# yuxiaoxiangyong/Multilateral-Temporal-view-Pyramid-Transformer-for-Video-Inpainting-Detection

Measured on AMD Instinct MI355X. Metric: clips/sec fwd (B=8,T=5,224x224), higher is better.
Workload: dtype f32; 1 GPU; full Mumpy forward (3 temporal views, pyramid decoder), B=8 clips/GPU, T=5, 224x224, fp32, tubelets (5,4,1); global_batch=8, launch=hipGraph replay, fork/join over HIP streams (independent branches co-scheduled), parallelism=batch-sharded x1, one metric all-reduce

## Files before the change

### multilateral-temporal-view-pyramid-transformer-for-video-inpainting-detection_amd/csrc/gemm.hip

```cpp
#include <stdlib.h>
#include "common.h"
#include "gemm_ws.h"
#include "gemm_ws64.h"
using namespace mumpy;

namespace {

constexpr int BK = 32;
constexpr int LDR = 36;

struct ConvGeom {
    int H, W, Cin, kh, kw, ph, pw;
    int kseg, kstride;
};

__device__ __attribute__((aligned(128))) float g_zero_page[32];

template <int TM, int TN, int WM, int WN, bool OUT16 = false>
__device__ __forceinline__ void store_tile(const f32x16 (&acc)[TM][TN], int64_t m0, int n0, int wm, int wn, int c, int h,
                                           int64_t M, int N, const float* __restrict__ bias, const float* residual,
                                           float* Y, int act, int ksplit, int ks, float* slab) {
    const int wm_u = __builtin_amdgcn_readfirstlane(wm), wn_u = __builtin_amdgcn_readfirstlane(wn);
    const int64_t mw = m0 + wm_u * WM;
    const int64_t wbase = mw * N + n0 + wn_u * WN;
// ... 429 lines not shown
                        acc[i][j] = __builtin_amdgcn_mfma_f32_32x32x16_bf16(af[i][st][NP > 1 ? PA[q] : 0],
                                                                            bf[j][st][NP > 1 ? PB[q] : 0], acc[i][j], 0, 0, 0);
    };
    const int klast = kbeg + (nk - 1) * BK;
    if (NBUF == 2) {
        gload(kbeg);
        lstore(0);
        __syncthreads();
        for (int kc = 0; kc + 1 < nk; ++kc) {
            gload(kbeg + (kc + 1) * BK);
            __builtin_amdgcn_sched_barrier(0);
            fread(kc & 1);
            mma();
            lstore((kc & 1) ^ 1);
            __syncthreads();
        }
        fread((nk - 1) & 1);
        mma();
    } else {
        gload(kbeg);
        lstore(0);
        gload(nk > 1 ? kbeg + BK : kbeg);
        __syncthreads();
        for (int kc = 0; kc + 1 < nk; ++kc) {
            fread(0);
            __syncthreads();
            lstore(0);
            const int knext = kbeg + (kc + 2) * BK;
            gload(knext < klast ? knext : klast);
            mma();
            __syncthreads();
        }
        fread(0);
        mma();
    }
    store_tile<TM, TN, WM, WN, OUT16>(acc, m0, n0, wm, wn, c, h, M, N, bias, residual, Y, act, ksplit, ks, slab);
}

__global__ __launch_bounds__(256) void splitk_reduce_kernel(const float* __restrict__ slab, const float* __restrict__ bias,
                                                            const float* residual, float* Y, int64_t MN4, int N,
                                                            int ksplit, int act) {
    for (int64_t i = (int64_t)blockIdx.x * 256 + threadIdx.x; i < MN4; i += (int64_t)gridDim.x * 256) {
        f32x4 v = ordered_sum(reinterpret_cast<const f32x4*>(slab)[i], reinterpret_cast<const f32x4*>(slab) + MN4 + i, MN4, ksplit - 1);
        const int n = (int)((i * 4) % N);
        if (bias) v += *reinterpret_cast<const f32x4*>(bias + n);
        if (act == MUMPY_ACT_GELU) {
#pragma unroll
            for (int e = 0; e < 4; ++e) v[e] = gelu_erf(v[e]);
        }
        if (residual) v += reinterpret_cast<const f32x4*>(residual)[i];
        reinterpret_cast<f32x4*>(Y)[i] = v;
    }
}

struct Plan {
    int tile;
    int ksplit;
    unsigned gn;
    int64_t gm;
};

constexpr int NUM_CU = 256;

Plan make_plan_x3(int64_t M, int N, int K, bool allow_split) {
    Plan p;
    const int64_t gm128 = (M + 127) / 128, gm64 = (M + 63) / 64;
    const unsigned gn128 = (N + 127) / 128, gn64 = (N + 63) / 64;
    const int64_t b128 = gm128 * gn128, b64 = gm64 * gn64;
    auto fit = [&](int ks) {
        if (!allow_split) return 1;
        if (ks > K / 384) ks = K / 384;
        if (ks > 16) ks = 16;
        while (ks > 1 && (K % (32 * ks)) != 0) --ks;
        return ks < 1 ? 1 : ks;
    };
    const int ksw = fit((int)((448 + b128 / 2) / b128));
    if (b128 * ksw >= 240) {
        p.tile = 0; p.ksplit = ksw; p.gm = gm128; p.gn = gn128;
    } else {
        p.tile = 2; p.ksplit = (b64 < 2 * 256 && K >= 768) ? fit((int)((3 * 256 + b64 - 1) / b64)) : 1;
        p.gm = gm64; p.gn = gn64;
    }
    return p;
}

Plan make_plan(int64_t M, int N, int K, bool allow_split, bool x3 = false) {
    static const char* force = tune_str("MUMPY_GEMM_FORCE");
    if (x3 && !force) return make_plan_x3(M, N, K, allow_split);
    Plan p;
    const int64_t gm128 = (M + 127) / 128, gm64 = (M + 63) / 64;
    const unsigned gn128 = (N + 127) / 128, gn64 = (N + 63) / 64;
    const int64_t b128 = gm128 * gn128, b64 = gm64 * gn64;
    const double nk = (double)K / BK;
    const double t128 = (double)((b128 + NUM_CU - 1) / NUM_CU) * (nk + 2.0) / nk;
    double t64 = (double)((b64 + NUM_CU - 1) / NUM_CU) * 0.272;
    if (t64 < 0.357) t64 = 0.357;
    t64 *= (nk + 0.5) / nk;
    int tile = (t128 <= t64) ? 0 : 2;
    if (tile == 0 && b128 > NUM_CU && K >= 512) tile = 3;
    int ks = 1;
    static const int min_slice = tune_int("MUMPY_GEMM_MINSLICE", 384), max_ks = tune_int("MUMPY_GEMM_MAXKS", 16),
                     min_k = tune_int("MUMPY_GEMM_SPLIT_MINK", 768);
    if (tile == 2 && allow_split && b64 < 2 * NUM_CU && K >= min_k) {
        ks = (int)((3 * NUM_CU + b64 - 1) / b64);
        if (ks > K / min_slice) ks = K / min_slice;
        if (ks > max_ks) ks = max_ks;
        while (ks > 1 && (K % (32 * ks)) != 0) --ks;
        if (ks < 1) ks = 1;
    }
    if (force) {
        int ft = -1, fk = -1;
        if (sscanf(force, "%d,%d", &ft, &fk) >= 1 && ft >= 0 && ft <= 3) {
            tile = ft;
            if (fk >= 1 && allow_split && K % (32 * fk) == 0) ks = fk; else if (fk >= 1) ks = 1;
        }
    }
    p.tile = tile; p.ksplit = ks;
    p.gm = (tile == 0 || tile == 3) ? gm128 : gm64;
    p.gn = (tile == 2) ? gn64 : gn128;
    return p;
}

int device_cus() {
    static int num_cu = 0;
    if (!num_cu) {
        int dev = 0;
        hipDeviceProp_t prop;
        if (hipGetDevice(&dev) == hipSuccess && hipGetDeviceProperties(&prop, dev) == hipSuccess) num_cu = prop.multiProcessorCount;
        else num_cu = NUM_CU;
    }
    return num_cu;
}

int ws_plan(int64_t M, int N, int K, bool have_ws, bool conv) {
    static const int ws_mode = tune_int("MUMPY_GEMM_WS", 2);
    const int num_cu = device_cus();
    const int64_t tiles = ((M + 127) / 128) * ((N + 127) / 128);
    const int nk = K / 32;
    const double rounds = (double)tiles / num_cu, eff = rounds / (double)((tiles + num_cu - 1) / num_cu);
    const double per_cu = (double)tiles * nk / num_cu;
    int how = 0;
    if (ws_mode == 1) how = 1;
    else if (ws_mode == 3) how = have_ws ? 2 : 1;
    else if (ws_mode == 2 && conv) {
        if (have_ws && eff < 0.86 && per_cu >= 24.0 && (double)nk / per_cu <= 3.0) how = 2;
        else if (tiles >= (int64_t)(0.75 * num_cu) && eff >= 0.75 && K >= 128) how = 1;
    } else if (ws_mode == 2) {
        if (tiles >= (int64_t)(0.75 * num_cu) && eff >= 0.86 && K >= 128 && !(K >= 1024 && rounds >= 1.8)) how = 1;
        else if (have_ws && eff < 0.86 && per_cu >= 24.0 && (double)nk / per_cu <= 3.0 && !(K >= 1024 && rounds >= 1.8)) how = 2;
    }
    return how;
}

int launch_linear(const float* x, const float* W, const float* bias, const float* residual, float* y, int64_t M, int N,
                  int K, int act, float* ws, int64_t ws_bytes, hipStream_t s, int64_t rpb = 0, int64_t bstride = 0,
                  const ConvGeom* conv = nullptr, bool ws_clean = false, const gemm_ws::LnArgs* ln = nullptr, int kseg = 0,
                  int kstride = 0) {
    if (rpb <= 0) { rpb = M; bstride = 0; }
    ConvGeom cg = conv ? *conv : ConvGeom{0, 0, 0, 0, 0, 0, 0, 0, 0};
    cg.kseg = kseg; cg.kstride = kstride;
    const bool math_bf16 = (act & MUMPY_MATH_BF16) != 0;
    const bool math_x2 = (act & MUMPY_MATH_BF16X2) != 0;
    const bool math_x3 = (act & MUMPY_MATH_BF16X3) != 0 || math_x2;
    act &= 0xff;
    const gemm_ws::Conv cvd{cg.H, cg.W, cg.Cin, cg.kh, cg.kw};
    if (ln && (rpb < M || math_bf16 || math_x3 || conv || !gemm_ws::eligible(M, N, K) ||
               !ws_plan(M, N, K, ws && ws_bytes >= gemm_ws::workspace_bytes(device_cus()), false))) {
        set_error("linear: LayerNorm folding needs a shape the persistent 128x128 kernel takes (mumpy_linear_ln_tiles) in fp32 mode");
        return MUMPY_EINVAL;
    }
    if (rpb >= M && !kseg && !math_bf16 && !math_x3 && (conv ? gemm_ws::conv_eligible(M, N, cvd) : gemm_ws::eligible(M, N, K))) {
        const int num_cu = device_cus();
        const bool have_ws = ws && ws_bytes >= gemm_ws::workspace_bytes(num_cu);
        const int how = ws_plan(M, N, K, have_ws, conv != nullptr);
        const int nk = K / 32;
        static const int ws64_mode = tune_int("MUMPY_GEMM_WS64", 1);
        if (!how && !conv && ws64_mode) {
            const int64_t t64 = ((M + 63) / 64) * ((N + 63) / 64);
            const double r64 = (double)t64 / (2.0 * num_cu);
            const bool fits = ws64_mode == 2 || (act != MUMPY_ACT_GELU && nk <= 32 && t64 >= 64 && (r64 <= 1.0 || r64 >= 2.5 || nk <= 12));
            if (fits) {
                if (int rc = gemm_ws64::launch(x, W, bias, residual, y, M, N, K, act, num_cu, s)) return rc;
                MUMPY_CHECK_LAUNCH("linear(ws64)");
                return 0;
            }
        }
        if (how) {
            if (int rc = gemm_ws::launch(x, W, bias, residual, y, M, N, K, act, num_cu, s, ws, ws_bytes, how == 2 ? 1 : 0, nullptr, ws_clean,
                                         conv ? &cvd : nullptr, ln)) return rc;
            MUMPY_CHECK_LAUNCH("linear(ws)");
            return 0;
        }
    }
    Plan p = make_plan(M, N, K, ws != nullptr, math_x3);
    if (ws) { ws += 1024; ws_bytes -= 4096; }
    if (p.ksplit > 1 && (int64_t)p.ksplit * M * N * (int64_t)sizeof(float) > ws_bytes) p.ksplit = 1;
    const int64_t grid = p.gm * p.gn * p.ksplit;
    MUMPY_REQUIRE(grid < (1ll << 31), MUMPY_ERANGE, "linear: too many tiles");
#define MUMPY_GEMM(BM_, BN_, WM_, WN_, CV_)                                                                        \
    if (use_glds)                                                                                                  \
        hipLaunchKernelGGL((linear_kernel<BM_, BN_, WM_, WN_, CV_, true>), dim3((unsigned)grid),                     \
                           dim3(64 * (BM_ / WM_) * (BN_ / WN_)), 0, s, x, W, bias, residual, y, M, N, K, act, p.gn,  \
                           p.ksplit, ws, rpb, bstride, cg);                                               \
    else                                                                                                           \
    hipLaunchKernelGGL((linear_kernel<BM_, BN_, WM_, WN_, CV_, false>), dim3((unsigned)grid),                        \
                       dim3(64 * (BM_ / WM_) * (BN_ / WN_)), 0, s, x, W, bias, residual, y, M, N, K, act, p.gn, p.ksplit, \
                       ws, rpb, bstride, cg)
    static const bool use_glds = tune_int("MUMPY_GEMM_GLDS", 0) != 0;
    if (math_x3) {
        const bool wide = (p.tile == 0 || p.tile == 3);
#define MUMPY_GEMM_X3(BM_, BN_, WM_, WN_, CV_, NB_)                                                                    \
    hipLaunchKernelGGL((linear_bf16_kernel<BM_, BN_, WM_, WN_, CV_, 3, NB_>), dim3((unsigned)grid), dim3(256), 0, s, x, W, \
                       bias, residual, y, M, N, K, act, p.gn, p.ksplit, ws, rpb, bstride, cg)
#define MUMPY_GEMM_X2(BM_, BN_, WM_, WN_, CV_, NB_)                                                                    \
    hipLaunchKernelGGL((linear_bf16_kernel<BM_, BN_, WM_, WN_, CV_, 2, NB_>), dim3((unsigned)grid), dim3(256), 0, s, x, W, \
                       bias, residual, y, M, N, K, act, p.gn, p.ksplit, ws, rpb, bstride, cg)
        if (math_x2) {
            if (wide && conv) MUMPY_GEMM_X2(128, 128, 64, 64, true, 1);
            else if (wide) MUMPY_GEMM_X2(128, 128, 64, 64, false, 1);
            else if (conv) MUMPY_GEMM_X2(64, 64, 32, 32, true, 2);
            else MUMPY_GEMM_X2(64, 64, 32, 32, false, 2);
        }
        else if (wide && conv) MUMPY_GEMM_X3(128, 128, 64, 64, true, 1);
        else if (wide) MUMPY_GEMM_X3(128, 128, 64, 64, false, 1);
        else if (conv) MUMPY_GEMM_X3(64, 64, 32, 32, true, 2);
        else MUMPY_GEMM_X3(64, 64, 32, 32, false, 2);
#undef MUMPY_GEMM_X3
#undef MUMPY_GEMM_X2
    } else if (math_bf16) {
        const bool wide = (p.tile == 0 || p.tile == 3);
#define MUMPY_GEMM_H(BM_, BN_, WM_, WN_, CV_)                                                                          \
    hipLaunchKernelGGL((linear_bf16_kernel<BM_, BN_, WM_, WN_, CV_>), dim3((unsigned)grid), dim3(256), 0, s, x, W, bias,   \
                       residual, y, M, N, K, act, p.gn, p.ksplit, ws, rpb, bstride, cg)
        if (wide && conv) MUMPY_GEMM_H(128, 128, 64, 64, true);
        else if (wide) MUMPY_GEMM_H(128, 128, 64, 64, false);
        else if (conv) MUMPY_GEMM_H(64, 64, 32, 32, true);
        else MUMPY_GEMM_H(64, 64, 32, 32, false);
#undef MUMPY_GEMM_H
    } else if (p.tile == 3) {
        if (conv)
            hipLaunchKernelGGL((linear_kernel<128, 128, 64, 64, true, true, false>), dim3((unsigned)grid), dim3(256), 0, s, x, W,
                               bias, residual, y, M, N, K, act, p.gn, p.ksplit, ws, rpb, bstride, cg);
        else
            hipLaunchKernelGGL((linear_kernel<128, 128, 64, 64, false, true, false>), dim3((unsigned)grid), dim3(256), 0, s, x, W,
                               bias, residual, y, M, N, K, act, p.gn, p.ksplit, ws, rpb, bstride, cg);
    } else if (conv) {
        if (p.tile == 0) MUMPY_GEMM(128, 128, 64, 32, true);
        else if (p.tile == 1) MUMPY_GEMM(64, 128, 32, 64, true);
        else MUMPY_GEMM(64, 64, 32, 32, true);
    } else {
        if (p.tile == 0) MUMPY_GEMM(128, 128, 64, 32, false);
        else if (p.tile == 1) MUMPY_GEMM(64, 128, 32, 64, false);
        else MUMPY_GEMM(64, 64, 32, 32, false);
    }
#undef MUMPY_GEMM
    MUMPY_CHECK_LAUNCH("linear");
    if (p.ksplit > 1) {
        const int64_t mn4 = M * N / 4;
        int64_t g = (mn4 + 255) / 256;
        if (g > 2048) g = 2048;
        hipLaunchKernelGGL(splitk_reduce_kernel, dim3((unsigned)g), dim3(256), 0, s, ws, bias, residual, y, mn4, N,
                           p.ksplit, act);
        MUMPY_CHECK_LAUNCH("linear(split-K reduce)");
    }
    return 0;
}

}

static int check_linear_args(const float* x, const float* W, const float* residual, const float* y, int64_t M, int N,
                             int K, int act) {
    MUMPY_REQUIRE(x && W && y, MUMPY_ENULL, "linear: null pointer");
    MUMPY_REQUIRE(aligned16(x) && aligned16(W) && aligned16(y) && aligned16(residual), MUMPY_EALIGN,
                  "linear: pointers must be 16-byte aligned");
    MUMPY_REQUIRE(M < (1ll << 31) - 256 && (int64_t)N * 4 * 128 < (1ll << 32), MUMPY_ERANGE,
                  "linear: M=%lld rows / N=%d columns beyond the 32-bit row index / tile byte offsets", (long long)M, N);
    MUMPY_REQUIRE(M >= 0 && N > 0 && K > 0 && K % BK == 0 && N % 32 == 0, MUMPY_EINVAL,
                  "linear: need K %% 32 == 0 and N %% 32 == 0 (got M=%lld N=%d K=%d)", (long long)M, N, K);
    MUMPY_REQUIRE((act & 0xff) == MUMPY_ACT_NONE || (act & 0xff) == MUMPY_ACT_GELU, MUMPY_EINVAL, "linear: unknown act %d", act);
    constexpr int math_bits = MUMPY_MATH_BF16 | MUMPY_MATH_BF16X3 | MUMPY_MATH_BF16X2;
    MUMPY_REQUIRE((act & ~(0xff | math_bits)) == 0, MUMPY_EINVAL, "linear: unknown flag bits in act 0x%x", act);
    MUMPY_REQUIRE(((act & math_bits) & ((act & math_bits) - 1)) == 0, MUMPY_EINVAL, "linear: the MUMPY_MATH_* modes are exclusive");
    return 0;
}

extern "C" int mumpy_linear_fwd(const float* x, const float* W, const float* bias, const float* residual, float* y,
                                int64_t M, int N, int K, int act, void* stream) {
    if (M == 0) return 0;
    if (int rc = check_linear_args(x, W, residual, y, M, N, K, act)) return rc;
    return launch_linear(x, W, bias, residual, y, M, N, K, act, nullptr, 0, as_stream(stream));
}

extern "C" int64_t mumpy_linear_workspace_bytes(int64_t M, int N, int K) {
    if (M <= 0 || N <= 0 || K <= 0 || K % BK) return 0;
    const Plan p = make_plan(M, N, K, true), q = make_plan(M, N, K, true, true);
    const int ks = p.ksplit > q.ksplit ? p.ksplit : q.ksplit;
    int64_t bytes = ks > 1 ? (int64_t)ks * M * N * (int64_t)sizeof(float) + 4096 : 0;
    if (gemm_ws::eligible(M, N, K)) {
        const int64_t tiles = ((M + 127) / 128) * ((N + 127) / 128);
        const double per_cu = (double)tiles * (K / 32) / NUM_CU;
        const int64_t need = gemm_ws::workspace_bytes(2 * NUM_CU);
        if (per_cu >= 16.0 && bytes < need) bytes = need;
    }
    return bytes;
}

extern "C" int mumpy_linear_ws_fwd(const float* x, const float* W, const float* bias, const float* residual, float* y,
                                   int64_t M, int N, int K, int act, void* workspace, int64_t workspace_bytes,
                                   void* stream) {
    if (M == 0) return 0;
    if (int rc = check_linear_args(x, W, residual, y, M, N, K, act)) return rc;
    MUMPY_REQUIRE(aligned16(workspace), MUMPY_EALIGN, "linear: workspace must be 16-byte aligned");
    return launch_linear(x, W, bias, residual, y, M, N, K, act, static_cast<float*>(workspace),
                         workspace ? workspace_bytes : 0, as_stream(stream));
}

extern "C" int mumpy_linear_bf16s_fwd(const void* x, const void* W, const float* bias, const float* residual, void* y,
                                      int64_t M, int N, int K, int act, int out_bf16, void* stream) {
    if (M == 0) return 0;
    MUMPY_REQUIRE(x && W && y, MUMPY_ENULL, "linear_bf16s: null pointer");
    MUMPY_REQUIRE(aligned16(x) && aligned16(W) && aligned16(y) && aligned16(residual), MUMPY_EALIGN,
                  "linear_bf16s: pointers must be 16-byte aligned");
    MUMPY_REQUIRE(M > 0 && M < (1ll << 31) - 256 && (int64_t)N * 4 * 128 < (1ll << 32), MUMPY_ERANGE, "linear_bf16s: M=%lld / N=%d out of range", (long long)M, N);
    MUMPY_REQUIRE(N > 0 && K > 0 && K % BK == 0 && N % 32 == 0, MUMPY_EINVAL, "linear_bf16s: need K %% 32 == 0 and N %% 32 == 0 (got N=%d K=%d)", N, K);
    MUMPY_REQUIRE(act == MUMPY_ACT_NONE || act == MUMPY_ACT_GELU, MUMPY_EINVAL, "linear_bf16s: unknown act %d", act);
    const float* xf = static_cast<const float*>(x);
    const float* wf = static_cast<const float*>(W);
    float* yf = static_cast<float*>(y);
    const ConvGeom cg{0, 0, 0, 0, 0, 0, 0, 0, 0};
    hipStream_t s = as_stream(stream);
    MUMPY_REQUIRE(!(out_bf16 && residual), MUMPY_EINVAL, "linear_bf16s: a bf16 output takes no residual");
    {
        static const int ws16 = tune_int("MUMPY_GEMM_WS16", 2);
        static int num_cu = 0;
        if (!num_cu) {
            int dev = 0;
            hipDeviceProp_t prop;
            if (hipGetDevice(&dev) == hipSuccess && hipGetDeviceProperties(&prop, dev) == hipSuccess) num_cu = prop.multiProcessorCount;
            else num_cu = NUM_CU;
        }
        const int64_t tiles = ((M + 127) / 128) * ((N + 127) / 128);
        const double rounds = (double)tiles / num_cu, eff = rounds / (double)((tiles + num_cu - 1) / num_cu);
        if (ws16 && gemm_ws::eligible16(M, N, K) && (ws16 == 2 || (tiles >= (int64_t)(0.75 * num_cu) && eff >= 0.75))) {
            if (int rc = gemm_ws::launch16(x, W, bias, residual, y, M, N, K, act, out_bf16 != 0, num_cu, s)) return rc;
            MUMPY_CHECK_LAUNCH("linear_bf16s(ws)");
            return 0;
        }
    }
    const int64_t gm128 = (M + 127) / 128, gm64 = (M + 63) / 64;
    const unsigned gn128 = (N + 127) / 128, gn64 = (N + 63) / 64;
    const bool wide = gm128 * gn128 >= 200;
    const unsigned gn = wide ? gn128 : gn64;
    const int64_t grid = (wide ? gm128 : gm64) * gn;
    MUMPY_REQUIRE(grid < (1ll << 31), MUMPY_ERANGE, "linear_bf16s: too many tiles");
#define MUMPY_GEMM_S(BM_, BN_, WM_, WN_, O16_)                                                                             \
    hipLaunchKernelGGL((linear_bf16_kernel<BM_, BN_, WM_, WN_, false, 1, 2, true, O16_>), dim3((unsigned)grid), dim3(256), 0, s, \
                       xf, wf, bias, residual, yf, M, N, K, act, gn, 1, nullptr, M, (int64_t)0, cg)
    if (wide && out_bf16) MUMPY_GEMM_S(128, 128, 64, 64, true);
    else if (wide) MUMPY_GEMM_S(128, 128, 64, 64, false);
    else if (out_bf16) MUMPY_GEMM_S(64, 64, 32, 32, true);
    else MUMPY_GEMM_S(64, 64, 32, 32, false);
#undef MUMPY_GEMM_S
    MUMPY_CHECK_LAUNCH("linear_bf16s");
    return 0;
}

extern "C" int mumpy_linear_wsz_fwd(const float* x, const float* W, const float* bias, const float* residual, float* y,
                                    int64_t M, int N, int K, int act, void* workspace, int64_t workspace_bytes,
                                    void* stream) {
    if (M == 0) return 0;
    if (int rc = check_linear_args(x, W, residual, y, M, N, K, act)) return rc;
    MUMPY_REQUIRE(aligned16(workspace), MUMPY_EALIGN, "linear: workspace must be 16-byte aligned");
    return launch_linear(x, W, bias, residual, y, M, N, K, act, static_cast<float*>(workspace),
                         workspace ? workspace_bytes : 0, as_stream(stream), 0, 0, nullptr, true);
}

extern "C" int mumpy_workspace_status(const void* workspace, int* status) {
    MUMPY_REQUIRE(workspace && status, MUMPY_ENULL, "workspace_status: null pointer");
    unsigned w[2] = {0, 0};
    static_assert(gemm_ws::LN_GUARD_WORD + 1 == gemm_ws::STATUS_WORD, "status words must be adjacent");
    hipError_t e = hipMemcpy(w, static_cast<const unsigned*>(workspace) + gemm_ws::LN_GUARD_WORD, sizeof(w), hipMemcpyDeviceToHost);
    if (e != hipSuccess) { set_error("workspace_status: %s", hipGetErrorString(e)); return (int)e; }
    *status = w[1] ? (int)w[1] : (w[0] ? -1 : 0);
    return 0;
}

extern "C" int mumpy_linear_ln_tiles(int64_t M, int N, int K) {
    if (M <= 0 || N <= 0 || K <= 0 || K % BK || N % 32 || !gemm_ws::eligible(M, N, K)) return 0;
    return ws_plan(M, N, K, true, false) ? (N + 127) / 128 : 0;
}

extern "C" int mumpy_linear_lnx_fwd(const float* x, const float* W, const float* bias, const float* residual, float* y, int64_t M,
                                    int N, int K, int act, void* workspace, int64_t workspace_bytes, float* stats_out,
                                    const float* ln_stats, int ln_gn, const float* ln_colsum, float ln_eps, void* stream) {
    if (M == 0) return 0;
    if (int rc = check_linear_args(x, W, residual, y, M, N, K, act)) return rc;
    MUMPY_REQUIRE((act & ~0xff) == 0, MUMPY_EINVAL, "linear_lnx: fp32 matrix math only");
    MUMPY_REQUIRE(aligned16(workspace) && workspace, MUMPY_EALIGN, "linear_lnx: needs the kept (zeroed) workspace of mumpy_linear_wsz_fwd");
    MUMPY_REQUIRE((stats_out != nullptr) != (ln_stats != nullptr), MUMPY_EINVAL, "linear_lnx: exactly one of stats_out (producer) / ln_stats (consumer)");
    MUMPY_REQUIRE(!ln_stats || (ln_colsum && bias && !residual && ln_gn == (K + 127) / 128 && ln_gn <= 16 && ln_eps > 0.f), MUMPY_EINVAL,
                  "linear_lnx: the consumer takes W gamma, colsum, bias = W beta + b, no residual, and ln_gn = ceil(K / 128) tiles (got %d)", ln_gn);
    MUMPY_REQUIRE(aligned16(stats_out) && aligned16(ln_stats) && aligned16(ln_colsum), MUMPY_EALIGN, "linear_lnx: pointers must be 16-byte aligned");
    MUMPY_REQUIRE(M * (int64_t)((N + 127) / 128) * 8 < (1ll << 31) && M * (int64_t)(ln_gn > 0 ? ln_gn : 1) * 8 < (1ll << 31), MUMPY_ERANGE,
                  "linear_lnx: statistics buffer beyond 2 GiB");
    const gemm_ws::LnArgs ln{stats_out, ln_stats, ln_colsum, ln_gn, K, ln_eps};
    return launch_linear(x, W, bias, residual, y, M, N, K, act, static_cast<float*>(workspace), workspace_bytes, as_stream(stream), 0, 0,
                         nullptr, true, &ln);
}

extern "C" int mumpy_linear_rows_fwd(const float* x, int64_t rows_per_block, int64_t block_stride, const float* W,
                                     const float* bias, const float* residual, float* y, int64_t M, int N, int K, int act,
                                     void* workspace, int64_t workspace_bytes, void* stream) {
    if (M == 0) return 0;
    if (int rc = check_linear_args(x, W, residual, y, M, N, K, act)) return rc;
    MUMPY_REQUIRE(rows_per_block > 0 && M % rows_per_block == 0 && block_stride % 4 == 0, MUMPY_EINVAL,
                  "linear_rows: M=%lld must be a multiple of rows_per_block=%lld and block_stride %% 4 == 0",
                  (long long)M, (long long)rows_per_block);
    return launch_linear(x, W, bias, residual, y, M, N, K, act, static_cast<float*>(workspace),
                         workspace ? workspace_bytes : 0, as_stream(stream), rows_per_block, block_stride);
}

extern "C" int mumpy_linear_rows_kseg_fwd(const float* x, int64_t rows_per_block, int64_t block_stride, int kseg, int kstride,
                                          const float* W, const float* bias, const float* residual, float* y, int64_t M, int N, int K,
                                          int act, void* workspace, int64_t workspace_bytes, void* stream) {
    if (M == 0) return 0;
    if (int rc = check_linear_args(x, W, residual, y, M, N, K, act)) return rc;
    MUMPY_REQUIRE(rows_per_block > 0 && M % rows_per_block == 0 && block_stride % 4 == 0, MUMPY_EINVAL,
                  "linear_rows_kseg: M=%lld must be a multiple of rows_per_block=%lld and block_stride %% 4 == 0",
                  (long long)M, (long long)rows_per_block);
    MUMPY_REQUIRE(kseg > 0 && kseg % 32 == 0 && K % kseg == 0 && kstride % 4 == 0 && kstride >= 0, MUMPY_EINVAL,
                  "linear_rows_kseg: need kseg %% 32 == 0, K %% kseg == 0, kstride %% 4 == 0 (got kseg=%d K=%d kstride=%d)", kseg, K, kstride);
    return launch_linear(x, W, bias, residual, y, M, N, K, act, static_cast<float*>(workspace), workspace ? workspace_bytes : 0,
                         as_stream(stream), rows_per_block, block_stride, nullptr, false, nullptr, kseg, kstride);
}

extern "C" int64_t mumpy_conv2d_workspace_bytes(int B, int H, int W, int Cin, int Cout, int kh, int kw) {
    return mumpy_linear_workspace_bytes((int64_t)B * H * W, Cout, kh * kw * Cin);
}

extern "C" int mumpy_conv2d_nhwc_fwd(const float* x, const float* w_krsc, const float* bias, const float* residual,
                                     float* y, int B, int H, int W, int Cin, int Cout, int kh, int kw, int act,
                                     void* workspace, int64_t workspace_bytes, void* stream) {
    MUMPY_REQUIRE(B > 0 && H > 0 && W > 0 && H < 32768 && W < 32768, MUMPY_EINVAL, "conv2d: bad image size %dx%d", H, W);
    MUMPY_REQUIRE(kh > 0 && kw > 0 && (kh & 1) && (kw & 1), MUMPY_EINVAL, "conv2d: kernel %dx%d must be odd (same padding)", kh, kw);
    MUMPY_REQUIRE(Cin % 32 == 0 && Cout % 32 == 0, MUMPY_EINVAL, "conv2d: Cin=%d and Cout=%d must be multiples of 32", Cin, Cout);
    const int64_t M = (int64_t)B * H * W;
    const int K = kh * kw * Cin;
    if (int rc = check_linear_args(x, w_krsc, residual, y, M, Cout, K, act)) return rc;
    MUMPY_REQUIRE(aligned16(workspace), MUMPY_EALIGN, "conv2d: workspace must be 16-byte aligned");
    const ConvGeom cg{H, W, Cin, kh, kw, kh / 2, kw / 2, 0, 0};
    return launch_linear(x, w_krsc, bias, residual, y, M, Cout, K, act, static_cast<float*>(workspace),
                         workspace ? workspace_bytes : 0, as_stream(stream), 0, 0, &cg);
}
```

### multilateral-temporal-view-pyramid-transformer-for-video-inpainting-detection_amd/csrc/gemm_ws64.h

```cpp
#pragma once
#include "gemm_ws.h"

namespace mumpy {
namespace gemm_ws64 {

using gemm_ws::BK;
using gemm_ws::OOB;
using gemm_ws::Params;
using gemm_ws::tile_coords;
using gemm_ws::u32x4;
using gemm_ws::ws_barrier;

constexpr int T = 64;
constexpr int STAGE_DW = 2 * T * BK;
constexpr int NSTAGE = 3;
constexpr int E_DW = T * T;
constexpr int E_OFF_DW = NSTAGE * STAGE_DW;
constexpr int LDS_BYTES = (E_OFF_DW + E_DW) * 4;
constexpr int PASSES = 4;

__device__ __forceinline__ void matrix_role(const Params& p, float* lds, int n_chunks, int wave, int lane) {
    const int c = lane & 31, h = lane >> 5, wm = wave >> 1, wn = wave & 1;
    const int sw = (c >> 1) & 7;
    int a_off[4], b_off[4];
#pragma unroll
    for (int q = 0; q < 4; ++q) {
        a_off[q] = (32 * wm + c) * BK + 4 * ((4 * h + q) ^ sw);
        b_off[q] = (T + 32 * wn + c) * BK + 4 * ((4 * h + q) ^ sw);
    }
    float* const E = lds + E_OFF_DW + (32 * wm + 4 * h) * T + 32 * wn + c;
    f32x16 acc;
    f32x4 fa0, fb0, fa1, fb1;
    auto rd = [&](const float* st, int q, f32x4& fa, f32x4& fb) {
        fa = *reinterpret_cast<const f32x4*>(st + a_off[q]);
        fb = *reinterpret_cast<const f32x4*>(st + b_off[q]);
    };
    auto mm = [&](const f32x4& fa, const f32x4& fb, int e) { acc = __builtin_amdgcn_mfma_f32_32x32x2f32(fa[e], fb[e], acc, 0, 0, 0); };
    auto mm4 = [&](const f32x4& fa, const f32x4& fb) {
#pragma unroll
        for (int e = 0; e < 4; ++e) mm(fa, fb, e);
    };
    auto dump = [&]() {
#pragma unroll
        for (int r = 0; r < 16; ++r) E[((r & 3) + 8 * (r >> 2)) * T] = acc[r];
    };
    auto zero = [&]() {
#pragma unroll
        for (int r = 0; r < 16; ++r) acc[r] = 0.f;
    };
    zero();
    ws_barrier();
    rd(lds, 0, fa0, fb0);
    int kc = 0, stage = 0;
    for (int i = 0; i < n_chunks; ++i) {
        const float* st = lds + stage * STAGE_DW;
        stage = stage == NSTAGE - 1 ? 0 : stage + 1;
        if (kc == 0 && i > 0) { dump(); zero(); }
        __builtin_amdgcn_sched_barrier(0);
        rd(st, 1, fa1, fb1);
        mm4(fa0, fb0);
        __builtin_amdgcn_sched_group_barrier(0x008, 1, 0);
        __builtin_amdgcn_sched_group_barrier(0x100, 2, 0);
        __builtin_amdgcn_sched_group_barrier(0x008, 3, 0);
        rd(st, 2, fa0, fb0);
        mm4(fa1, fb1);
        __builtin_amdgcn_sched_group_barrier(0x008, 1, 0);
        __builtin_amdgcn_sched_group_barrier(0x100, 2, 0);
        __builtin_amdgcn_sched_group_barrier(0x008, 3, 0);
        rd(st, 3, fa1, fb1);
        mm4(fa0, fb0);
        __builtin_amdgcn_sched_group_barrier(0x008, 1, 0);
        __builtin_amdgcn_sched_group_barrier(0x100, 2, 0);
        __builtin_amdgcn_sched_group_barrier(0x008, 3, 0);
        mm(fa1, fb1, 0);
        mm(fa1, fb1, 1);
        __builtin_amdgcn_sched_barrier(0);
        ws_barrier();
        __builtin_amdgcn_sched_barrier(0);
        rd(lds + stage * STAGE_DW, 0, fa0, fb0);
        mm(fa1, fb1, 2);
        mm(fa1, fb1, 3);
        __builtin_amdgcn_sched_barrier(0);
        if (++kc == p.nk) kc = 0;
    }
    dump();
    ws_barrier();
}

__device__ __forceinline__ void loader_role(const Params& p, float* lds, unsigned tile0, int n_chunks, int hl) {
    const int lane = hl & 63, lw = __builtin_amdgcn_readfirstlane(hl >> 6);
    const int prow = lane >> 3;
    uint32_t aoff[2], boff[2];
    auto set_tile = [&](unsigned t) {
        unsigned tm, tn;
        tile_coords(p, t, tm, tn);
#pragma unroll
        for (int q = 0; q < 2; ++q) {
            const int r = 32 * q + 8 * lw + prow;
            const uint32_t ch = (uint32_t)((lane & 7) ^ ((r >> 1) & 7));
            int m = (int)tm * T + r;
            if (m > p.M - 1) m = p.M - 1;
            aoff[q] = (uint32_t)m * (uint32_t)p.K * 4u + 16u * ch;
            int n = (int)tn * T + r;
            if (n > p.N - 1) n = p.N - 1;
            boff[q] = (uint32_t)n * (uint32_t)p.K * 4u + 16u * ch;
        }
    };
    const auto rs_x = __builtin_amdgcn_make_buffer_rsrc(const_cast<float*>(p.X), 0, (int)0x7fffffff, 0x00020000);
    const auto rs_w = __builtin_amdgcn_make_buffer_rsrc(const_cast<float*>(p.W), 0, (int)0x7fffffff, 0x00020000);
    typedef __attribute__((address_space(3))) void* lptr_t;
    auto dma = [&](int kc, int stage) {
        const int so = kc * 128;
        float* st = lds + stage * STAGE_DW + 8 * lw * BK;
#pragma unroll
        for (int q = 0; q < 2; ++q)
            __builtin_amdgcn_raw_ptr_buffer_load_lds(rs_x, (lptr_t)(st + 32 * q * BK), 16, aoff[q], so, 0, 0);
#pragma unroll
        for (int q = 0; q < 2; ++q)
            __builtin_amdgcn_raw_ptr_buffer_load_lds(rs_w, (lptr_t)(st + (T + 32 * q) * BK), 16, boff[q], so, 0, 0);
    };
    unsigned ld_tile = tile0;
    int ld_kc = 0, ld_idx = 0;
    auto advance = [&]() {
        if (ld_idx + 1 < n_chunks) {
            ++ld_idx;
            if (++ld_kc == p.nk) { ld_kc = 0; ++ld_tile; set_tile(ld_tile); }
        }
    };
    set_tile(ld_tile);
    dma(ld_kc, 0);
    advance();
    dma(ld_kc, 1);
    advance();
    asm volatile("s_waitcnt vmcnt(4)" ::: "memory");
    ws_barrier();
    int stage = 2;
    for (int i = 0; i < n_chunks; ++i) {
        dma(ld_kc, stage);
        advance();
        stage = stage == NSTAGE - 1 ? 0 : stage + 1;
        asm volatile("s_waitcnt vmcnt(4)" ::: "memory");
        ws_barrier();
    }
    asm volatile("s_waitcnt vmcnt(0)" ::: "memory");
    ws_barrier();
}

template <int P>
__device__ __forceinline__ void epilogue_role(const Params& p, float* lds, unsigned v0, unsigned n_tiles, int hl) {
    const float* const E = lds + E_OFF_DW;
    const int e_row = hl >> 4, e_c4 = hl & 15;
    const int nk = p.nk;
    const auto rs_y = __builtin_amdgcn_make_buffer_rsrc(p.Y, 0, (int)((int64_t)p.M * p.N * 4), 0x00020000);
    const auto rs_r = __builtin_amdgcn_make_buffer_rsrc(const_cast<float*>(p.residual ? p.residual : p.Y), 0,
                                                        p.residual ? (int)((int64_t)p.M * p.N * 4) : 0, 0x00020000);
    const auto rs_b = __builtin_amdgcn_make_buffer_rsrc(const_cast<float*>(p.bias ? p.bias : p.Y), 0, p.bias ? p.N * 4 : 0, 0x00020000);
    constexpr int STEPS = PASSES / P;
    f32x4 rv[PASSES], bias4;
    uint32_t yo[PASSES];
    const uint32_t row16 = 16u * (uint32_t)p.N * 4u;
    auto begin_tile = [&](unsigned t) {
        unsigned tm, tn;
        tile_coords(p, t, tm, tn);
        const int n = (int)tn * T + 4 * e_c4;
        const uint32_t ybase = n < p.N ? (((uint32_t)tm * T + e_row) * (uint32_t)p.N + (uint32_t)n) * 4u : OOB;
#pragma unroll
        for (int e = 0; e < PASSES; ++e) {
            yo[e] = ybase + (uint32_t)e * row16;
            rv[e] = __builtin_bit_cast(f32x4, __builtin_amdgcn_raw_buffer_load_b128(rs_r, yo[e], 0, 0));
        }
        bias4 = __builtin_bit_cast(f32x4, __builtin_amdgcn_raw_buffer_load_b128(rs_b, n < p.N ? (uint32_t)n * 4u : OOB, 0, 0));
    };
    auto pass = [&](int e) {
        f32x4 v = *reinterpret_cast<const f32x4*>(E + (16 * e + e_row) * T + 4 * e_c4) + bias4;
        if (p.act == MUMPY_ACT_GELU) {
#pragma unroll
            for (int x = 0; x < 4; ++x) v[x] = gelu_erf(v[x]);
        }
        v += rv[e];
        __builtin_amdgcn_raw_buffer_store_b128(__builtin_bit_cast(u32x4, v), rs_y, yo[e], 0, 0);
    };
    ws_barrier();
    for (int c = 0; c < nk; ++c) ws_barrier();
    for (unsigned t = 1; t < n_tiles; ++t) {
        begin_tile(v0 + t - 1);
        ws_barrier();
#pragma unroll
        for (int st = 0; st < STEPS; ++st) {
#pragma unroll
            for (int k = 0; k < P; ++k) pass(st * P + k);
            ws_barrier();
        }
        for (int c = 1 + STEPS; c < nk; ++c) ws_barrier();
    }
    begin_tile(v0 + n_tiles - 1);
    ws_barrier();
#pragma unroll
    for (int e = 0; e < PASSES; ++e) pass(e);
}

template <int P>
__global__ __launch_bounds__(768, 6) void gemm_ws64_kernel(Params p) {
    extern __shared__ __attribute__((aligned(1024))) float lds[];
    const int tid = threadIdx.x, lane = tid & 63;
    const int wave = __builtin_amdgcn_readfirstlane(tid >> 6);
    const unsigned G = gridDim.x, orig = blockIdx.x, xcd = orig & 7, q8 = G >> 3, r8 = G & 7;
    const unsigned b = (xcd < r8 ? xcd * (q8 + 1) : r8 * (q8 + 1) + (xcd - r8) * q8) + (orig >> 3);
    const unsigned cnt = b < p.tiles ? (p.tiles - b + G - 1) / G : 0;
    if (cnt == 0) return;
    const unsigned v0 = b * p.rr_cnt;
    const int n_chunks = (int)cnt * p.nk;
    if (wave < 4) matrix_role(p, lds, n_chunks, wave, lane);
    else {
        __builtin_amdgcn_s_setprio(3);
        if (wave < 8) loader_role(p, lds, v0, n_chunks, tid - 256);
        else epilogue_role<P>(p, lds, v0, cnt, tid - 512);
    }
}

inline bool eligible(int64_t M, int N, int K) { return gemm_ws::eligible(M, N, K); }

inline int launch(const float* x, const float* W, const float* bias, const float* residual, float* y, int64_t M, int N, int K,
                  int act, int num_cu, hipStream_t s, int per_cu = 2) {
    Params p;
    p.cv_H = p.cv_W = p.cv_C = p.cv_kh = p.cv_kw = p.cv_cpc = 0;
    p.cv_mhw = p.cv_shw = p.cv_mw = p.cv_sw = 0;
    p.X = x; p.W = W; p.bias = bias; p.residual = residual; p.Y = y;
    p.M = (int)M; p.N = N; p.K = K; p.act = act; p.nk = K / BK;
    p.gm = (unsigned)((M + T - 1) / T); p.gn = (unsigned)((N + T - 1) / T);
    p.tiles = p.gm * p.gn;
    p.units = p.tiles * (unsigned)p.nk;
#ifdef MUMPY_WS_STAMP
    p.stamps = nullptr;
#endif
    const int need = (PASSES + p.nk - 2) / (p.nk - 1);
    const int P = need <= 1 ? 1 : need <= 2 ? 2 : 4;
    p.lmin = 0;
    const unsigned slots = (unsigned)per_cu * (unsigned)num_cu;
    const int lds_bytes = per_cu == 1 ? 2 * LDS_BYTES + 1024 : LDS_BYTES;
    const unsigned grid = p.tiles < slots ? p.tiles : slots;
    p.st_w = (p.gn % 4 == 0) ? 4u : (p.gn % 2 == 0) ? 2u : 1u;
    p.rr_G = grid;
    p.rr_cnt = (p.tiles + grid - 1) / grid;
    p.flags = nullptr; p.slabs = nullptr;
#define MUMPY_WS64_LAUNCH(P_)                                                                                           \
    do {                                                                                                                \
        static bool attr_set = false;                                                                                   \
        if (!attr_set) {                                                                                                \
            hipError_t e = hipFuncSetAttribute(reinterpret_cast<const void*>(gemm_ws64_kernel<P_>),                     \
                                               hipFuncAttributeMaxDynamicSharedMemorySize, 2 * LDS_BYTES + 1024);       \
            if (e != hipSuccess) { set_error("gemm_ws64: cannot reserve %d B of LDS: %s", 2 * LDS_BYTES + 1024, hipGetErrorString(e)); return (int)e; } \
            attr_set = true;                                                                                            \
        }                                                                                                               \
        hipLaunchKernelGGL(gemm_ws64_kernel<P_>, dim3(grid), dim3(768), lds_bytes, s, p);                               \
    } while (0)
    if (P == 1) MUMPY_WS64_LAUNCH(1);
    else if (P == 2) MUMPY_WS64_LAUNCH(2);
    else MUMPY_WS64_LAUNCH(4);
#undef MUMPY_WS64_LAUNCH
    return 0;
}

}
}
```

Measured before the change: 372.6 clips/s.

## Add stream-K split mode to 64x64 warp-specialized GEMM with slab fixup

Extends the 64x64 persistent warp-specialized GEMM so work can be split at K-chunk granularity across workgroups (stream-K). Partial tiles are written to workspace slabs and signalled with flags, and the tile owner spins on those flags and reduces the partials before the epilogue. A cost model picks split versus whole-tile scheduling. The eligibility policy also changes so GELU GEMMs can use ws64, with a tunable per-CU occupancy. The split path adds memset, spin-wait and slab traffic, and relies on the workspace being large enough.

```diff
diff --git a/multilateral-temporal-view-pyramid-transformer-for-video-inpainting-detection_amd/csrc/gemm.hip b/multilateral-temporal-view-pyramid-transformer-for-video-inpainting-detection_amd/csrc/gemm.hip
--- a/multilateral-temporal-view-pyramid-transformer-for-video-inpainting-detection_amd/csrc/gemm.hip
+++ b/multilateral-temporal-view-pyramid-transformer-for-video-inpainting-detection_amd/csrc/gemm.hip
@@ -605,6 +605,36 @@
     return how;
 }
 
+struct Ws64Plan { bool use, split; int per_cu, min_p; };
+Ws64Plan ws64_plan(int64_t M, int N, int K, int act, int num_cu, int64_t ws_bytes, int mode) {
+    Ws64Plan q{false, false, 2, 2};
+    const int64_t tiles = ((M + 63) / 64) * ((N + 63) / 64);
+    const int64_t nk = K / 32;
+    const bool gelu = act == MUMPY_ACT_GELU;
+    if (mode == 4 || (mode == 1 && !gelu)) {
+        const double r64 = (double)tiles / (2.0 * num_cu);
+        q.use = !gelu && nk <= 32 && tiles >= 64 && (r64 <= 1.0 || r64 >= 2.5 || nk <= 12);
+        return q;
+    }
+    if (mode == 1 && nk > 24) return q;
+    static const int gelu_per_cu = tune_int("MUMPY_WS64_GELU_PERCU", 1), min_p = tune_int("MUMPY_WS64_MINP", 2);
+    q.use = true;
+    q.per_cu = gelu ? gelu_per_cu : 2;
+    q.min_p = min_p;
+    const int64_t slots = (int64_t)q.per_cu * num_cu;
+    const bool can_split = slots <= gemm_ws64::MAX_SPLIT_GRID && ws_bytes >= gemm_ws64::workspace_bytes((int)slots);
+    if (mode == 2 || !can_split) return q;
+    if (mode == 3) { q.split = true; return q; }
+    const double rate = q.per_cu >= 2 ? 1.0 : 1.1;
+    const int64_t gw = tiles < slots ? tiles : slots;
+    const double wg_per_cu_w = (double)((gw + num_cu - 1) / num_cu);
+    const double whole = wg_per_cu_w * (double)((tiles + gw - 1) / gw) * (double)nk * (wg_per_cu_w >= 2 ? 1.0 : 1.1) + 3.0;
+    const int64_t lmin = 1 + 4 / (q.min_p >= 4 ? 4 : 2);
+    const double split = (double)q.per_cu * (double)((tiles * nk + slots - 1) / slots + (lmin - 1 > 2 ? lmin - 1 : 2)) * rate + 3.0 + 4.0;
+    q.split = split < whole;
+    return q;
+}
+
 int launch_linear(const float* x, const float* W, const float* bias, const float* residual, float* y, int64_t M, int N,
                   int K, int act, float* ws, int64_t ws_bytes, hipStream_t s, int64_t rpb = 0, int64_t bstride = 0,
                   const ConvGeom* conv = nullptr, bool ws_clean = false, const gemm_ws::LnArgs* ln = nullptr, int kseg = 0,
@@ -626,14 +656,12 @@
         const int num_cu = device_cus();
         const bool have_ws = ws && ws_bytes >= gemm_ws::workspace_bytes(num_cu);
         const int how = ws_plan(M, N, K, have_ws, conv != nullptr);
-        const int nk = K / 32;
         static const int ws64_mode = tune_int("MUMPY_GEMM_WS64", 1);
         if (!how && !conv && ws64_mode) {
-            const int64_t t64 = ((M + 63) / 64) * ((N + 63) / 64);
-            const double r64 = (double)t64 / (2.0 * num_cu);
-            const bool fits = ws64_mode == 2 || (act != MUMPY_ACT_GELU && nk <= 32 && t64 >= 64 && (r64 <= 1.0 || r64 >= 2.5 || nk <= 12));
-            if (fits) {
-                if (int rc = gemm_ws64::launch(x, W, bias, residual, y, M, N, K, act, num_cu, s)) return rc;
+            const Ws64Plan q = ws64_plan(M, N, K, act, num_cu, ws ? ws_bytes : 0, ws64_mode);
+            if (q.use) {
+                if (int rc = gemm_ws64::launch(x, W, bias, residual, y, M, N, K, act, num_cu, s, q.per_cu, ws, ws_bytes, q.split,
+                                               ws_clean, q.min_p)) return rc;
                 MUMPY_CHECK_LAUNCH("linear(ws64)");
                 return 0;
             }
@@ -754,6 +782,11 @@
         const double per_cu = (double)tiles * (K / 32) / NUM_CU;
         const int64_t need = gemm_ws::workspace_bytes(2 * NUM_CU);
         if (per_cu >= 16.0 && bytes < need) bytes = need;
+        const int64_t need64 = gemm_ws64::workspace_bytes(gemm_ws64::MAX_SPLIT_GRID);
+        const int mode = tune_int("MUMPY_GEMM_WS64", 1);
+        if (bytes < need64 && (ws64_plan(M, N, K, MUMPY_ACT_NONE, NUM_CU, need64, mode).split ||
+                               ws64_plan(M, N, K, MUMPY_ACT_GELU, NUM_CU, need64, mode).split))
+            bytes = need64;
     }
     return bytes;
 }
diff --git a/multilateral-temporal-view-pyramid-transformer-for-video-inpainting-detection_amd/csrc/gemm_ws64.h b/multilateral-temporal-view-pyramid-transformer-for-video-inpainting-detection_amd/csrc/gemm_ws64.h
--- a/multilateral-temporal-view-pyramid-transformer-for-video-inpainting-detection_amd/csrc/gemm_ws64.h
+++ b/multilateral-temporal-view-pyramid-transformer-for-video-inpainting-detection_amd/csrc/gemm_ws64.h
@@ -19,7 +19,7 @@
 constexpr int LDS_BYTES = (E_OFF_DW + E_DW) * 4;
 constexpr int PASSES = 4;
 
-__device__ __forceinline__ void matrix_role(const Params& p, float* lds, int n_chunks, int wave, int lane) {
+__device__ __forceinline__ void matrix_role(const Params& p, float* lds, int kc0, int n_chunks, int wave, int lane) {
     const int c = lane & 31, h = lane >> 5, wm = wave >> 1, wn = wave & 1;
     const int sw = (c >> 1) & 7;
     int a_off[4], b_off[4];
@@ -51,7 +51,7 @@
     zero();
     ws_barrier();
     rd(lds, 0, fa0, fb0);
-    int kc = 0, stage = 0;
+    int kc = kc0, stage = 0;
     for (int i = 0; i < n_chunks; ++i) {
         const float* st = lds + stage * STAGE_DW;
         stage = stage == NSTAGE - 1 ? 0 : stage + 1;
@@ -87,7 +87,7 @@
     ws_barrier();
 }
 
-__device__ __forceinline__ void loader_role(const Params& p, float* lds, unsigned tile0, int n_chunks, int hl) {
+__device__ __forceinline__ void loader_role(const Params& p, float* lds, unsigned tile0, int kc0, int n_chunks, int hl) {
     const int lane = hl & 63, lw = __builtin_amdgcn_readfirstlane(hl >> 6);
     const int prow = lane >> 3;
     uint32_t aoff[2], boff[2];
@@ -120,7 +120,7 @@
             __builtin_amdgcn_raw_ptr_buffer_load_lds(rs_w, (lptr_t)(st + (T + 32 * q) * BK), 16, boff[q], so, 0, 0);
     };
     unsigned ld_tile = tile0;
-    int ld_kc = 0, ld_idx = 0;
+    int ld_kc = kc0, ld_idx = 0;
     auto advance = [&]() {
         if (ld_idx + 1 < n_chunks) {
             ++ld_idx;
@@ -147,14 +147,16 @@
 }
 
 template <int P>
-__device__ __forceinline__ void epilogue_role(const Params& p, float* lds, unsigned v0, unsigned n_tiles, int hl) {
+__device__ __forceinline__ void epilogue_role(const Params& p, float* lds, unsigned b, unsigned G, unsigned u0, unsigned u1, int hl) {
     const float* const E = lds + E_OFF_DW;
     const int e_row = hl >> 4, e_c4 = hl & 15;
-    const int nk = p.nk;
+    const unsigned nk = (unsigned)p.nk;
+    const bool split = p.flags != nullptr;
     const auto rs_y = __builtin_amdgcn_make_buffer_rsrc(p.Y, 0, (int)((int64_t)p.M * p.N * 4), 0x00020000);
     const auto rs_r = __builtin_amdgcn_make_buffer_rsrc(const_cast<float*>(p.residual ? p.residual : p.Y), 0,
                                                         p.residual ? (int)((int64_t)p.M * p.N * 4) : 0, 0x00020000);
     const auto rs_b = __builtin_amdgcn_make_buffer_rsrc(const_cast<float*>(p.bias ? p.bias : p.Y), 0, p.bias ? p.N * 4 : 0, 0x00020000);
+    const auto rs_s = __builtin_amdgcn_make_buffer_rsrc(split ? p.slabs + (size_t)b * E_DW : p.Y, 0, split ? E_DW * 4 : 0, 0x00020000);
     constexpr int STEPS = PASSES / P;
     f32x4 rv[PASSES], bias4;
     uint32_t yo[PASSES];
@@ -180,10 +182,43 @@
         v += rv[e];
         __builtin_amdgcn_raw_buffer_store_b128(__builtin_bit_cast(u32x4, v), rs_y, yo[e], 0, 0);
     };
-    ws_barrier();
-    for (int c = 0; c < nk; ++c) ws_barrier();
-    for (unsigned t = 1; t < n_tiles; ++t) {
-        begin_tile(v0 + t - 1);
+    const uint32_t soff = ((uint32_t)e_row * T + 4u * e_c4) * 4u;
+    auto pass_part = [&](int e) {
+        const f32x4 v = *reinterpret_cast<const f32x4*>(E + (16 * e + e_row) * T + 4 * e_c4);
+        __builtin_amdgcn_raw_buffer_store_b128(__builtin_bit_cast(u32x4, v), rs_s, soff, e * (16 * T * 4), 0);
+    };
+    auto publish = [&]() {
+        if (hl == 0) {
+            __builtin_amdgcn_fence(__ATOMIC_RELEASE, "agent");
+            asm volatile("s_waitcnt vmcnt(0)" ::: "memory");
+            __hip_atomic_store(p.flags + b, 1u, __ATOMIC_RELAXED, __HIP_MEMORY_SCOPE_AGENT);
+        }
+    };
+
+    ws_barrier();
+    unsigned prev_t = u0 / nk;
+    bool prev_part = (u0 % nk) != 0;
+    unsigned u = (prev_t + 1) * nk < u1 ? (prev_t + 1) * nk : u1;
+    for (unsigned c = u0; c < u; ++c) ws_barrier();
+    if (u < u1 && prev_part) {
+        const unsigned end = u + nk < u1 ? u + nk : u1;
+        ws_barrier();
+#pragma unroll
+        for (int st = 0; st < STEPS; ++st) {
+#pragma unroll
+            for (int k = 0; k < P; ++k) pass_part(st * P + k);
+            if (st == STEPS - 1) asm volatile("s_waitcnt vmcnt(0)" ::: "memory");
+            ws_barrier();
+        }
+        publish();
+        for (unsigned c = u + 1 + STEPS; c < end; ++c) ws_barrier();
+        prev_t = u / nk;
+        prev_part = false;
+        u = end;
+    }
+    while (u < u1) {
+        const unsigned end = u + nk < u1 ? u + nk : u1;
+        begin_tile(prev_t);
         ws_barrier();
 #pragma unroll
         for (int st = 0; st < STEPS; ++st) {
@@ -191,10 +226,54 @@
             for (int k = 0; k < P; ++k) pass(st * P + k);
             ws_barrier();
         }
-        for (int c = 1 + STEPS; c < nk; ++c) ws_barrier();
-    }
-    begin_tile(v0 + n_tiles - 1);
-    ws_barrier();
+        for (unsigned c = u + 1 + STEPS; c < end; ++c) ws_barrier();
+        prev_t = u / nk;
+        u = end;
+    }
+    const bool head = split && !prev_part && (u1 % nk) != 0;
+    if (!prev_part) begin_tile(prev_t);
+    ws_barrier();
+    if (prev_part) {
+#pragma unroll
+        for (int e = 0; e < PASSES; ++e) pass_part(e);
+        asm volatile("s_waitcnt vmcnt(0)\n\ts_barrier" ::: "memory");
+        publish();
+        return;
+    }
+    if (head) {
+        const unsigned tile_end = (prev_t + 1) * nk;
+        if (hl == 0) {
+            for (unsigned b2 = b + 1; b2 < G; ++b2) {
+                const unsigned f0 = gemm_ws::first_chunk(b2, G, p.units, p.nk, p.lmin);
+                if (f0 >= tile_end) break;
+                if (gemm_ws::first_chunk(b2 + 1, G, p.units, p.nk, p.lmin) == f0) continue;
+                unsigned spins = 0;
+                while (__hip_atomic_load(p.flags + b2, __ATOMIC_RELAXED, __HIP_MEMORY_SCOPE_AGENT) == 0u && ++spins < (1u << 24))
+                    __builtin_amdgcn_s_sleep(8);
+                if (spins >= (1u << 24)) {
+                    __hip_atomic_store(p.flags + gemm_ws::STATUS_WORD, 1u + b2, __ATOMIC_RELAXED, __HIP_MEMORY_SCOPE_AGENT);
+                    continue;
+                }
+                __hip_atomic_store(p.flags + b2, 0u, __ATOMIC_RELAXED, __HIP_MEMORY_SCOPE_AGENT);
+            }
+            __builtin_amdgcn_fence(__ATOMIC_ACQUIRE, "agent");
+            asm volatile("s_waitcnt vmcnt(0)" ::: "memory");
+        }
+        asm volatile("s_waitcnt vmcnt(0) lgkmcnt(0)\n\ts_barrier" ::: "memory");
+        float* const Ew = lds + E_OFF_DW;
+        for (unsigned b2 = b + 1; b2 < G; ++b2) {
+            const unsigned f0 = gemm_ws::first_chunk(b2, G, p.units, p.nk, p.lmin);
+            if (f0 >= tile_end) break;
+            if (gemm_ws::first_chunk(b2 + 1, G, p.units, p.nk, p.lmin) == f0) continue;
+            const float* sl = p.slabs + (size_t)b2 * E_DW + e_row * T + 4 * e_c4;
+#pragma unroll
+            for (int e = 0; e < PASSES; ++e) {
+                f32x4* d = reinterpret_cast<f32x4*>(Ew + (16 * e + e_row) * T + 4 * e_c4);
+                *d += *reinterpret_cast<const f32x4*>(sl + 16 * e * T);
+            }
+        }
+        asm volatile("s_waitcnt lgkmcnt(0)" ::: "memory");
+    }
 #pragma unroll
     for (int e = 0; e < PASSES; ++e) pass(e);
 }
@@ -206,43 +285,71 @@
     const int wave = __builtin_amdgcn_readfirstlane(tid >> 6);
     const unsigned G = gridDim.x, orig = blockIdx.x, xcd = orig & 7, q8 = G >> 3, r8 = G & 7;
     const unsigned b = (xcd < r8 ? xcd * (q8 + 1) : r8 * (q8 + 1) + (xcd - r8) * q8) + (orig >> 3);
-    const unsigned cnt = b < p.tiles ? (p.tiles - b + G - 1) / G : 0;
-    if (cnt == 0) return;
-    const unsigned v0 = b * p.rr_cnt;
-    const int n_chunks = (int)cnt * p.nk;
-    if (wave < 4) matrix_role(p, lds, n_chunks, wave, lane);
+    const unsigned nk = (unsigned)p.nk;
+    unsigned u0, u1;
+    if (p.flags != nullptr) {
+        u0 = gemm_ws::first_chunk(b, G, p.units, p.nk, p.lmin);
+        u1 = gemm_ws::first_chunk(b + 1, G, p.units, p.nk, p.lmin);
+    } else {
+        const unsigned cnt = b < p.tiles ? (p.tiles - b + G - 1) / G : 0;
+        u0 = b * p.rr_cnt * nk;
+        u1 = u0 + cnt * nk;
+    }
+    const int n_chunks = (int)(u1 - u0);
+    if (n_chunks == 0) return;
+    const unsigned t0 = u0 / nk;
+    const int kc0 = (int)(u0 - t0 * nk);
+    if (wave < 4) gemm_ws64::matrix_role(p, lds, kc0, n_chunks, wave, lane);
     else {
         __builtin_amdgcn_s_setprio(3);
-        if (wave < 8) loader_role(p, lds, v0, n_chunks, tid - 256);
-        else epilogue_role<P>(p, lds, v0, cnt, tid - 512);
+        if (wave < 8) gemm_ws64::loader_role(p, lds, t0, kc0, n_chunks, tid - 256);
+        else gemm_ws64::epilogue_role<P>(p, lds, b, G, u0, u1, tid - 512);
     }
 }
 
 inline bool eligible(int64_t M, int N, int K) { return gemm_ws::eligible(M, N, K); }
 
+constexpr int MAX_SPLIT_GRID = gemm_ws::LN_GUARD_WORD;
+inline int64_t workspace_bytes(int grid) { return 4096 + (int64_t)grid * E_DW * 4; }
+
 inline int launch(const float* x, const float* W, const float* bias, const float* residual, float* y, int64_t M, int N, int K,
-                  int act, int num_cu, hipStream_t s, int per_cu = 2) {
+                  int act, int num_cu, hipStream_t s, int per_cu = 2, void* ws = nullptr, int64_t ws_bytes = 0, bool split = false,
+                  bool ws_clean = false, int min_p = 2) {
     Params p;
     p.cv_H = p.cv_W = p.cv_C = p.cv_kh = p.cv_kw = p.cv_cpc = 0;
     p.cv_mhw = p.cv_shw = p.cv_mw = p.cv_sw = 0;
+    p.stats_out = nullptr; p.ln_stats = nullptr; p.ln_colsum = nullptr; p.ln_gn = p.ln_C = 0; p.ln_eps = 0.f; p.ln_guard = nullptr;
     p.X = x; p.W = W; p.bias = bias; p.residual = residual; p.Y = y;
     p.M = (int)M; p.N = N; p.K = K; p.act = act; p.nk = K / BK;
     p.gm = (unsigned)((M + T - 1) / T); p.gn = (unsigned)((N + T - 1) / T);
     p.tiles = p.gm * p.gn;
     p.units = p.tiles * (unsigned)p.nk;
+    p.walk = 0u;
 #ifdef MUMPY_WS_STAMP
     p.stamps = nullptr;
 #endif
+    const unsigned slots = (unsigned)per_cu * (unsigned)num_cu;
+    if (split && (slots > (unsigned)MAX_SPLIT_GRID || !ws || ws_bytes < workspace_bytes((int)slots))) split = false;
     const int need = (PASSES + p.nk - 2) / (p.nk - 1);
-    const int P = need <= 1 ? 1 : need <= 2 ? 2 : 4;
-    p.lmin = 0;
-    const unsigned slots = (unsigned)per_cu * (unsigned)num_cu;
+    int P = need <= 1 ? 1 : need <= 2 ? 2 : 4;
+    if (split && P < min_p) P = min_p >= 4 ? 4 : 2;
+    p.lmin = 1 + PASSES / P;
     const int lds_bytes = per_cu == 1 ? 2 * LDS_BYTES + 1024 : LDS_BYTES;
-    const unsigned grid = p.tiles < slots ? p.tiles : slots;
+    unsigned grid = p.tiles < slots ? p.tiles : slots;
     p.st_w = (p.gn % 4 == 0) ? 4u : (p.gn % 2 == 0) ? 2u : 1u;
     p.rr_G = grid;
     p.rr_cnt = (p.tiles + grid - 1) / grid;
     p.flags = nullptr; p.slabs = nullptr;
+    if (split) {
+        grid = slots;
+        p.rr_cnt = 0;
+        p.flags = static_cast<unsigned*>(ws);
+        p.slabs = reinterpret_cast<float*>(static_cast<char*>(ws) + 4096);
+        if (!ws_clean) {
+            hipError_t e = hipMemsetAsync(p.flags, 0, 4096, s);
+            if (e != hipSuccess) { set_error("gemm_ws64: flag reset failed: %s", hipGetErrorString(e)); return (int)e; }
+        }
+    }
 #define MUMPY_WS64_LAUNCH(P_)                                                                                           \
     do {                                                                                                                \
         static bool attr_set = false;                                                                                   \
```

New measurement: 371.6 clips/s, median of 2. No clear change (-0.3%).
